# PolarisRisingWar/rgb-experiment

Hardware: AMD Instinct MI355X
Metric: aggregated edges/sec (full-graph GCN d=128, reference epoch = train fwd+bwd+Adam + 2 eval fwd) (higher is better)
Workload: dtype f32

## Files before the change

include/rgbx_hip.h:

```cpp
#ifndef RGBX_HIP_H
#define RGBX_HIP_H

#include <stddef.h>
#include <stdint.h>

#ifdef __cplusplus
extern "C" {
#endif

#define RGBX_VERSION 501

#define RGBX_OK 0
#define RGBX_E_ARG (-1)
#define RGBX_E_RANGE (-2)
#define RGBX_E_ALIGN (-3)
#define RGBX_E_WS (-4)
#define RGBX_E_SHAPE (-5)

typedef void* rgbx_stream_t;

enum {
  RGBX_LOOPS_KEEP = 0,
  RGBX_LOOPS_ADD_REMAINING = 1,
  RGBX_LOOPS_REMOVE_ADD = 2
// ... 100 lines not shown

typedef struct rgbx_spmm_epilogue {
  const struct rgbx_ce_epilogue* ce;
  int64_t n_classes;
  double* out_colsums;
  void* stats_ws;
  size_t stats_ws_bytes;
} rgbx_spmm_epilogue_t;

int rgbx_spmm_csr_epilogue_supported(int64_t d);
int rgbx_spmm_csr_epilogue_f32(const int32_t* rowptr, const int32_t* col, const float* w, const float* rs,
                               const float* x, int64_t ldx, const float* y, int64_t ldy, const float* bias,
                               float* out, int64_t ldo, int64_t N, int64_t d, float a, float b,
                               const rgbx_row_split_t* split, const rgbx_spmm_epilogue_t* epi,
                               rgbx_stream_t stream);

int rgbx_spmm_csr_short_rows_supported(int64_t d);
int rgbx_spmm_csr_short_rows_f32(const int32_t* rowptr, const int32_t* col, const float* w, const float* x, int64_t ldx,
                                 const float* bias, float* out, int64_t ldo, int64_t N, int64_t d, rgbx_stream_t stream);

typedef struct rgbx_ce_epilogue {
  const int64_t* y;
  const uint8_t* mask;
  const float* grad_scale;
  double* stats;
  double* scratch;
  int32_t mask_groups;
  const int32_t* rows;
  int64_t n_rows;
  int32_t skip_unselected;
} rgbx_ce_epilogue_t;

int rgbx_spmm_linear_supported(int64_t K, int64_t Nout, int has_root);
int rgbx_spmm_linear_stats_workspace_bytes(int64_t N, int64_t Nout, size_t* bytes);
int rgbx_spmm_linear_f32(const int32_t* rowptr, const int32_t* col, const float* w, const float* rs,
                         const float* x, int64_t ldx, const float* wt, const float* x_root, int64_t ldr,
                         const float* wt_root, const float* bias, float* out, int64_t ldo, float* z_out,
                         int64_t ldz, const float* pre_scale, const float* pre_shift, const float* pre_rowsum,
                         double* out_colsums, void* stats_ws, size_t stats_ws_bytes,
                         const rgbx_ce_epilogue_t* ce, int64_t N, int64_t K, int64_t Nout,
                         const rgbx_row_split_t* split, rgbx_stream_t stream);

typedef struct rgbx_fused_layer {
  const int32_t* rowptr;
  const int32_t* col;
  const float* w;
  const float* rs;
  const float* x;
  int64_t ldx;
  int64_t x_blk_cols, x_blk_stride;
  const float* wt;
  const float* x_root;
  int64_t ldr;
  int64_t xr_blk_cols, xr_blk_stride;
  const float* wt_root;
  const float* bias;
  float* out;
  int64_t ldo;
  float* out_blk;
  int64_t ob_cols, ob_stride;
  float* z_out;
  int64_t ldz;
  const float* pre_scale;
  const float* pre_shift;
  const float* pre_rowsum;
  double* out_colsums;
// ... 293 lines not shown
```

rgb_experiment_amd/_lib.py:

```python
import ctypes
import os

import torch

_HERE = os.path.dirname(os.path.abspath(__file__))
LIB_PATH = os.path.join(_HERE, "csrc", "librgbx_hip.so")

_P = ctypes.c_void_p
_I64 = ctypes.c_int64
_I = ctypes.c_int
_F = ctypes.c_float

class RowSplit(ctypes.Structure):
    _fields_ = [("threshold", ctypes.c_int32), ("n_chunks", ctypes.c_int32), ("n_long", ctypes.c_int32),
                ("chunk_begin", ctypes.c_void_p), ("chunk_end", ctypes.c_void_p), ("chunk_row", ctypes.c_void_p),
                ("long_row", ctypes.c_void_p),
                ("long_chunk_ptr", ctypes.c_void_p), ("partial", ctypes.c_void_p)]


class MultiOut(ctypes.Structure):
    _fields_ = [(f, t) for name in ("sum", "mean", "var", "std", "max", "argmax", "min", "argmin")
                for f, t in ((name, ctypes.c_void_p), ("ld_" + name, ctypes.c_int64))]


# ... 19 lines not shown
                ("xr_blk_cols", _I64), ("xr_blk_stride", _I64), ("wt_root", _P), ("bias", _P), ("out", _P),
                ("ldo", _I64), ("out_blk", _P), ("ob_cols", _I64), ("ob_stride", _I64), ("z_out", _P), ("ldz", _I64),
                ("pre_scale", _P), ("pre_shift", _P), ("pre_rowsum", _P), ("out_colsums", _P), ("stats_ws", _P),
                ("stats_ws_bytes", ctypes.c_size_t), ("ce", _P), ("N", _I64), ("K", _I64), ("Nout", _I64),
                ("split", _P), ("w_pos", _P), ("z_pos_out", _P), ("col_sel", _P)]


SIGNATURES = {
    "rgbx_csr_workspace_bytes": [_I64, _I64, ctypes.POINTER(ctypes.c_size_t)],
    "rgbx_csr_build": [_P, _P, _I64, _I64, _I, _P, _P, _P, _P, ctypes.c_size_t, _P],
    "rgbx_deg_inv_sqrt_f32": [_P, _I64, _P, _P],
    "rgbx_gcn_norm_f32": [_P, _P, _I64, _P, _P, _P],
    "rgbx_inv_degree_f32": [_P, _I64, _P, _P],
    "rgbx_loop_weights_f32": [_P, _P, _P, _I64, _I64, _I, _F, _P, _P, _P],
    "rgbx_edge_slot_weights_f32": [_P, _I64, _P, _I64, _P, _P, _P],
    "rgbx_weighted_deg_inv_sqrt_f32": [_P, _P, _I64, _P, _P],
    "rgbx_gcn_norm_weighted_f32": [_P, _P, _P, _I64, _P, _P, _P],
    "rgbx_edge_dot_supported": [_I64],
    "rgbx_edge_dot_f32": [_P, _P, _P, _I64, _P, _I64, _P, _I64, _I64, _P, _P],
    "rgbx_gcn_norm_bwd_f32": [_P, _P, _P, _P, _P, _P, _P, _P, _P, _P, _I64, _I64, _P, _P, _P],
    "rgbx_spmm_csr_f32": [_P, _P, _P, _P, _P, _I64, _P, _I64, _P, _P, _I64, _I64, _I64, _F, _F, _P, _P],
    "rgbx_spmm_csr_extremum_supported": [_I64],
    "rgbx_spmm_csr_extremum_f32": [_P, _P, _P, _I64, _P, _I64, _P, _I64, _I64, _I, _P, _P],
    "rgbx_extremum_bwd_f32": [_P, _P, _P, _P, _I64, _P, _P, _I64, _I64, _I64, _P, _P],
    "rgbx_spmm_csr_multi_supported": [_I64],
    "rgbx_spmm_csr_multi_partial_words": [_I64, _I64, _I, ctypes.POINTER(ctypes.c_int64)],
    "rgbx_spmm_csr_multi_f32": [_P, _P, _P, _I64, _P, _I64, _I64, _P, _P],
    "rgbx_multi_bwd_f32": [_P, _P, _P, _P, _P, _I64, _I64, _I64, _P, _P],
    "rgbx_spmm_csr_epilogue_supported": [_I64],
    "rgbx_spmm_csr_epilogue_f32": [_P, _P, _P, _P, _P, _I64, _P, _I64, _P, _P, _I64, _I64, _I64, _F, _F, _P, _P, _P],
    "rgbx_spmm_csr_short_rows_supported": [_I64],
    "rgbx_spmm_csr_short_rows_f32": [_P, _P, _P, _P, _I64, _P, _P, _I64, _I64, _I64, _P],
    "rgbx_spmm_linear_supported": [_I64, _I64, _I],
    "rgbx_spmm_linear_stats_workspace_bytes": [_I64, _I64, ctypes.POINTER(ctypes.c_size_t)],
    "rgbx_spmm_linear_f32": [_P, _P, _P, _P, _P, _I64, _P, _P, _I64, _P, _P, _P, _I64, _P, _I64, _P, _P, _P, _P, _P,
                             ctypes.c_size_t, _P, _I64, _I64, _I64, _P, _P],
    "rgbx_fused_layer_f32": [_P, _P],
    "rgbx_blocked_to_rows_f32": [_P, _I64, _I64, _P, _I64, _I64, _I64, _P, _P],
    "rgbx_appnp_f32": [_P, _P, _P, _P, _I64, _P, _P, _I64, _I64, _I64, _I, _F, _P, _P],
    "rgbx_dagnn_gate_fwd_f32": [_P, _I64, _P, _I64, _I64, _P, _P, _P, _I64, _I64, _I64, _I, _P],
    "rgbx_dagnn_gate_bwd_workspace_bytes": [_I64, ctypes.POINTER(ctypes.c_size_t)],
    "rgbx_dagnn_gate_bwd_f32": [_P, _I64, _P, _I64, _I64, _P, _P, _P, _I64, _P, _I64, _P, _I64, _I64, _P, _P, _P,
                                ctypes.c_size_t, _I64, _I64, _I, _P],
    "rgbx_gru_step_supported": [_I64],
    "rgbx_gru_step_f32": [_P, _P, _P, _I64, _P, _P, _P, _P, _I64, _P, _I64, _P, _I64, _I64, _I64, _P, _P],
    "rgbx_gru_gate_fwd_f32": [_P, _I64, _P, _I64, _P, _I64, _I64, _I64, _P],
    "rgbx_gru_gate_bwd_f32": [_P, _I64, _P, _I64, _P, _I64, _P, _I64, _P, _I64, _I64, _I64, _P],
    "rgbx_gat_scores_f32": [_P, _I64, _P, _P, _P, _P, _I64, _I, _I, _P],
    "rgbx_gat_scores_bwd_scratch_floats": [_I64, _I, _I, ctypes.POINTER(ctypes.c_int64)],
    "rgbx_gat_scores_bwd_f32": [_P, _I64, _P, _P, _I64, _P, _P, _P, _I64, _P, _P, _P, _I64, _I64, _I, _I, _P],
    "rgbx_gat_aggregate_fwd_f32": [_P, _P, _P, _I64, _P, _P, _P, _P, _P, _P, _P, _I64, _P, _P, _P, _P, _I64, _I, _I, _F, _P,
                                   _P],
    "rgbx_gat_edge_softmax_f32": [_P, _P, _P, _P, _F, _P, _P, _P, _P, _P, _I64, _P, _P],
    "rgbx_gat_bwd_dst_f32": [_P, _P, _P, _I64, _P, _P, _P, _P, _P, _I64, _P, _I64, _P, _P, _I64, _I, _I,
                             _F, _P],
    "rgbx_gat_bwd_prep_f32": [_P, _P, _P, _P, _I64, _P, _P, _I64, _P, _P, _P, _F, _P, _I64, _I, _I, _P],
    "rgbx_gat_bwd_src_f32": [_P, _P, _P, _I64, _P, _P, _P, _I64, _P, _I64, _P, _P, _P, _P, _I64, _I, _I, _F, _P, _P],
    "rgbx_supergat_supported": [_I, _I],
    "rgbx_supergat_loss_records": [_I64, _P, ctypes.POINTER(ctypes.c_int64)],
    "rgbx_supergat_aggregate_fwd_f32": [_P, _P, _P, _I64, _P, _P, _P, _P, _I64, _P, _P, _I64, _I, _I, _F, _P, _F, _F, _P,
                                        _I64, _P, _P, _P],
    "rgbx_supergat_bwd_dst_f32": [_P, _P, _P, _I64, _P, _P, _P, _P, _P, _I64, _P, _P, _I64, _P, _P, _I64, _P, _I64, _I, _I,
                                  _F, _P, _F, _F, _P, _P, _P],
    "rgbx_supergat_bwd_src_f32": [_P, _P, _P, _P, _I64, _P, _P, _P, _I64, _P, _I64, _P, _I64, _I, _I, _F, _P, _F, _F, _P,
                                  _P, _P],
    "rgbx_supergat_sample_negatives": [_P, _I64, _I64, _P, _I64, _I, _P, _P, _P],
# ... 122 lines not shown
```

rgb_experiment_amd/csrc/gemm.hip:

```cpp
#include "rgbx_common.h"

namespace rgbx {
namespace {

constexpr int BM = 128, BN = 128, KT = 32;
enum { A_PLAIN = 0, A_BN = 1, A_ROWS = 2 };

struct TnExtra {
  const float* X;
  int64_t ldx;
  const float *mean, *rstd, *ca, *cb, *ck;
  const int32_t* rows;
  int64_t n_rows;
};
using f32x16 = __attribute__((ext_vector_type(16))) float;

template <int W>
__device__ __forceinline__ void stage_tile(float* __restrict__ lds, const float* __restrict__ src,
                                           int64_t ld, int64_t k0, int64_t k_end, int c0, int ncols) {
  const int tid = threadIdx.x;
#pragma unroll 4
  for (int p = 0; p < KT * W / 256; ++p) {
    const int idx = p * 256 + tid;
    const int r = idx / W, c = idx % W;
// ... 20 lines not shown
#pragma unroll
  for (int p = 0; p < KT * (W / 4) / 256; ++p) {
    const int idx = p * 256 + threadIdx.x;
    const int r = idx / (W / 4), c = (idx % (W / 4)) * 4;
    *reinterpret_cast<float4*>(lds + r * W + c) = regs[p];
  }
}

template <int W>
__device__ __forceinline__ void put_tile_bn(float* __restrict__ lds, const float4 (&rg)[KT * (W / 4) / 256],
                                            const float4 (&rx)[KT * (W / 4) / 256], const float* __restrict__ lc,
                                            int64_t k0, int64_t k_end, int c0, int ncols) {
#pragma unroll
  for (int p = 0; p < KT * (W / 4) / 256; ++p) {
    const int idx = p * 256 + threadIdx.x;
    const int r = idx / (W / 4), c = (idx % (W / 4)) * 4;
    float4 v = rg[p];
    if (k0 + r < k_end && c0 + c < ncols) {
      const float4 mu = *reinterpret_cast<const float4*>(lc + 0 * W + c);
      const float4 rs = *reinterpret_cast<const float4*>(lc + 1 * W + c);
      const float4 a = *reinterpret_cast<const float4*>(lc + 2 * W + c);
      const float4 b = *reinterpret_cast<const float4*>(lc + 3 * W + c);
      const float4 k = *reinterpret_cast<const float4*>(lc + 4 * W + c);
      v.x = bn_bwd_input_grad(v.x, rx[p].x, mu.x, rs.x, a.x, b.x, k.x);
      v.y = bn_bwd_input_grad(v.y, rx[p].y, mu.y, rs.y, a.y, b.y, k.y);
      v.z = bn_bwd_input_grad(v.z, rx[p].z, mu.z, rs.z, a.z, b.z, k.z);
      v.w = bn_bwd_input_grad(v.w, rx[p].w, mu.w, rs.w, a.w, b.w, k.w);
    }
    *reinterpret_cast<float4*>(lds + r * W + c) = v;
  }
}

template <int W>
__device__ __forceinline__ void fetch_tile_rows(float4 (&regs)[KT * (W / 4) / 256], const float* __restrict__ src,
                                                int64_t ld, const int32_t* __restrict__ rows, int64_t j0, int64_t j_end,
                                                int c0, int ncols) {
#pragma unroll
  for (int p = 0; p < KT * (W / 4) / 256; ++p) {
    const int idx = p * 256 + threadIdx.x;
    const int r = idx / (W / 4), c = (idx % (W / 4)) * 4;
    const int64_t j = j0 + r;
    regs[p] = make_float4(0.f, 0.f, 0.f, 0.f);
    if (j < j_end && c0 + c < ncols) regs[p] = *reinterpret_cast<const float4*>(src + (int64_t)rows[j] * ld + c0 + c);
  }
}

__device__ __forceinline__ int64_t lower_bound_rows(const int32_t* __restrict__ rows, int64_t n, int64_t key) {
  int64_t lo = 0, hi = n;
  while (lo < hi) {
    const int64_t mid = (lo + hi) >> 1;
    if (rows[mid] < key) lo = mid + 1; else hi = mid;
  }
  return lo;
}

template <bool VEC4, int MT, int MODE = A_PLAIN>
__global__ void __launch_bounds__(256)
gemm_tn_partial_kernel(const float* __restrict__ A, int64_t lda, const float* __restrict__ B, int64_t ldb,
                       float* __restrict__ part, float* __restrict__ colpart, int64_t K, int M, int N,
                       int64_t slab, TnExtra ex) {
  static_assert(MODE == A_PLAIN || VEC4, "the A_BN / A_ROWS forms exist on the 16-byte path only");
  constexpr int MI = MT / 64;
  __shared__ float lds[KT * (MT + 128) + (MODE == A_BN ? 5 * MT : 0)];
  float* la = lds;
  float* lb = lds + KT * MT;
  const int split = blockIdx.x;
  const int m0 = blockIdx.y * MT, n0 = blockIdx.z * BN;
  const int64_t k_begin = (int64_t)split * slab;
  const int64_t k_end = k_begin + slab < K ? k_begin + slab : K;
  const int wave = threadIdx.x >> 6, lane = threadIdx.x & 63;
  const int wm = (wave >> 1) * (MT / 2), wn = (wave & 1) * 64;
  const int kr = lane >> 5, cc = lane & 31;

  f32x16 acc[MI][2];
#pragma unroll
  for (int i = 0; i < MI; ++i)
// ... 20 lines not shown
      for (int i = 0; i < MI; ++i) {
        acc[i][0] = __builtin_amdgcn_mfma_f32_32x32x2f32(a[i], b0, acc[i][0], 0, 0, 0);
        acc[i][1] = __builtin_amdgcn_mfma_f32_32x32x2f32(a[i], b1, acc[i][1], 0, 0, 0);
      }
    }
  };
  if constexpr (MODE == A_BN) {
    float* lc = lds + KT * (MT + 128);
    for (int i = threadIdx.x; i < 5 * MT; i += 256) {
      const float* src = i < MT ? ex.mean : i < 2 * MT ? ex.rstd : i < 3 * MT ? ex.ca : i < 4 * MT ? ex.cb : ex.ck;
      const int c = m0 + i % MT;
      lc[i] = c < M ? src[c] : 0.f;
    }
    float4 ra[KT * (MT / 4) / 256], rx[KT * (MT / 4) / 256], rb[KT * 32 / 256];
    fetch_tile<MT>(ra, A, lda, k_begin, k_end, m0, M);
    fetch_tile<MT>(rx, ex.X, ex.ldx, k_begin, k_end, m0, M);
    fetch_tile<128>(rb, B, ldb, k_begin, k_end, n0, N);
    for (int64_t k0 = k_begin; k0 < k_end; k0 += KT) {
      __syncthreads();
      put_tile_bn<MT>(la, ra, rx, lc, k0, k_end, m0, M);
      put_tile<128>(lb, rb);
      __syncthreads();
      if (k0 + KT < k_end) {
        fetch_tile<MT>(ra, A, lda, k0 + KT, k_end, m0, M);
        fetch_tile<MT>(rx, ex.X, ex.ldx, k0 + KT, k_end, m0, M);
        fetch_tile<128>(rb, B, ldb, k0 + KT, k_end, n0, N);
      }
      consume();
    }
  } else if constexpr (MODE == A_ROWS) {
    const int64_t j_begin = lower_bound_rows(ex.rows, ex.n_rows, k_begin);
    const int64_t j_end = lower_bound_rows(ex.rows, ex.n_rows, k_end);
    float4 ra[KT * (MT / 4) / 256], rb[KT * 32 / 256];
    fetch_tile_rows<MT>(ra, A, lda, ex.rows, j_begin, j_end, m0, M);
    fetch_tile_rows<128>(rb, B, ldb, ex.rows, j_begin, j_end, n0, N);
    for (int64_t j0 = j_begin; j0 < j_end; j0 += KT) {
      __syncthreads();
      put_tile<MT>(la, ra);
      put_tile<128>(lb, rb);
      __syncthreads();
      if (j0 + KT < j_end) {
        fetch_tile_rows<MT>(ra, A, lda, ex.rows, j0 + KT, j_end, m0, M);
        fetch_tile_rows<128>(rb, B, ldb, ex.rows, j0 + KT, j_end, n0, N);
      }
      consume();
    }
  } else if constexpr (VEC4) {
    float4 ra[KT * (MT / 4) / 256], rb[KT * 32 / 256];
    fetch_tile<MT>(ra, A, lda, k_begin, k_end, m0, M);
    fetch_tile<128>(rb, B, ldb, k_begin, k_end, n0, N);
    for (int64_t k0 = k_begin; k0 < k_end; k0 += KT) {
      __syncthreads();
      put_tile<MT>(la, ra);
      put_tile<128>(lb, rb);
      __syncthreads();
      if (k0 + KT < k_end) {
        fetch_tile<MT>(ra, A, lda, k0 + KT, k_end, m0, M);
        fetch_tile<128>(rb, B, ldb, k0 + KT, k_end, n0, N);
      }
      consume();
    }
  } else {
    for (int64_t k0 = k_begin; k0 < k_end; k0 += KT) {
      __syncthreads();
      stage_tile<MT>(la, A, lda, k0, k_end, m0, M);
      stage_tile<128>(lb, B, ldb, k0, k_end, n0, N);
      __syncthreads();
      consume();
    }
  }

  if (sums && m0 + (int)threadIdx.x < M) colpart[(int64_t)split * M + m0 + threadIdx.x] = csum;
  float* out = part + (int64_t)split * M * N;
#pragma unroll
  for (int i = 0; i < MI; ++i)
#pragma unroll
// ... 140 lines not shown
```

rgb_experiment_amd/csrc/spmm_linear.hip:

```cpp
#include "rgbx_common.h"
#include "spmm_internal.h"

namespace rgbx {
namespace {

using f32x16 = __attribute__((ext_vector_type(16))) float;

using f4v = __attribute__((ext_vector_type(4))) float;
__device__ __forceinline__ void nt_store4(float* p, const float (&v)[4]) {
  f4v t = {v[0], v[1], v[2], v[3]};
  __builtin_nontemporal_store(t, reinterpret_cast<f4v*>(p));
}
__device__ __forceinline__ void nt_store1(float* p, float v) { __builtin_nontemporal_store(v, p); }

struct FusedArgs {
  const int* rowptr;
  const int* col;
  const float* w;
  const float* rs;
  const float* x;
  const float* wt;
  const float* xr;
  const float* wtr;
  const float* bias;
  float* out;
  float* z_out;
  int64_t ldx, ldo, ldz, ldr;
  const int* long_row;
  const float* zlong;
  int threshold, n_long;
  int N, K, Nout;
  const float* pre_scale;
  const float* pre_shift;
  const float* pre_rowsum;
  float* stats_part;
  const int64_t* ce_y;
  const uint8_t* ce_mask;
  const float* ce_scale;
  double* ce_part;
  int ce_groups;
  int64_t x_bc, x_bs, xr_bc, xr_bs;
  float* out_blk;
  int64_t ob_c, ob_s;
  const float* w2;
  float* zpos_out;
  const float* zlong_pos;
  const int* ce_rows;
  int ce_n_rows;
  int ce_skip;
  const uint8_t* col_sel;
};

__device__ __forceinline__ const float* blocked_at(const float* base, int64_t bc, int64_t bs, int64_t ld, int row,
                                                   int c) {
  return bc ? base + (int64_t)(c / (int)bc) * bs + (int64_t)row * bc + (c % (int)bc) : base + (int64_t)row * ld + c;
}

constexpr int TM = kTileRows;
constexpr int NT_ROOT = 2;

constexpr int KB = 16;

__device__ __forceinline__ void load_b_batch(float (&b)[KB], const float* __restrict__ wt, int Nout, int n0,
                                             int s0, int kr, int cc) {
#pragma unroll
  for (int i = 0; i < KB; ++i) b[i] = wt[(int64_t)(2 * (s0 + i) + kr) * Nout + n0 + cc];
}

__device__ __forceinline__ void mfma_batch(f32x16& acc, const float (&b)[KB], const float* __restrict__ zt, int ldz,
                                           int s0, int kr, int cc) {
#pragma unroll
  for (int i = 0; i < KB; ++i) {
    const float a = zt[cc * ldz + 2 * (s0 + i) + kr];
    acc = __builtin_amdgcn_mfma_f32_32x32x2f32(a, b[i], acc, 0, 0, 0);
  }
}

template <int KC>
__device__ __forceinline__ void tile_times_wt(f32x16& acc, const float* __restrict__ zt, int ldz,
                                              const float* __restrict__ wt, int K, int Nout, int n0, int kr,
                                              int cc, const float (*first)[KB] = nullptr) {
  if constexpr (KC > 0) {
// ... 98 lines not shown
    for (int b = q; b < G; b += 32) s += part2[(int64_t)b * width2 + c];
  sh[q][j] = s;
  __syncthreads();
  if (q == 0 && c < width2) {
    double t = 0.0;
#pragma unroll
    for (int k = 0; k < 32; ++k) t += sh[k][j];
    sums[c] = t;
  }
}


__device__ __forceinline__ int ce_select(const FusedArgs& A, int row, int* t) {
  int bits = A.ce_mask ? (int)A.ce_mask[row] : 1;
  bits = A.ce_groups == 2 ? (bits & 3) : (bits ? 1 : 0);
  *t = -1;
  if (bits) {
    const int64_t ti = A.ce_y[row];
    if (ti >= 0 && ti < A.Nout) *t = (int)ti;
  }
  return *t >= 0 ? bits : 0;
}

template <bool CE>
__device__ __forceinline__ int tile_row(const FusedArgs& A, int row_base, int r) {
  if constexpr (CE) {
    if (A.ce_rows) {
      const int i = row_base + r;
      const int row = i < A.ce_n_rows ? A.ce_rows[i] : A.N;
      return (unsigned)row < (unsigned)A.N ? row : A.N;
    }
  }
  return row_base + r;
}

__device__ __forceinline__ void ce_epilogue(const FusedArgs& A, const f32x16& acc, float* __restrict__ ot, int row_base,
                                            int wave, int lane, int tile = -1) {
  if (tile < 0) tile = blockIdx.x;
  const int kr = lane >> 5, cc = lane & 31;
  const int ldq = A.Nout + 4;
  const int n0 = wave * 32;
  __syncthreads();
  if (n0 < A.Nout) {
    const float bb = A.bias ? A.bias[n0 + cc] : 0.f;
#pragma unroll
    for (int r = 0; r < 16; ++r) ot[((r & 3) + 8 * (r >> 2) + 4 * kr) * ldq + n0 + cc] = acc[r] + bb;
  }
  __syncthreads();
  double nll = 0.0, nll2 = 0.0;
  int cnt = 0, hit = 0, cnt2 = 0, hit2 = 0;
  const int W = 3 * A.ce_groups;
  const float sc = A.ce_scale ? A.ce_scale[0] : 0.f;
  const bool c0 = lane < A.Nout, c1 = lane + 64 < A.Nout;
  for (int rr = 0; rr < TM / 4; ++rr) {
    const int rl = wave * (TM / 4) + rr;
    const int row = tile_row<true>(A, row_base, rl);
    if (row >= A.N) break;
    int t;
    const int bits = ce_select(A, row, &t);
    if (t < 0 && !A.ce_scale) continue;
    const float v0 = c0 ? ot[rl * ldq + lane] : -INFINITY;
    const float v1 = c1 ? ot[rl * ldq + lane + 64] : -INFINITY;
    float best = v0;
    int arg = c0 ? lane : INT32_MAX;
    if (v1 > best) { best = v1; arg = lane + 64; }
#pragma unroll
    for (int off = 32; off > 0; off >>= 1) {
      const float ob = __shfl_xor(best, off);
      const int oa = __shfl_xor(arg, off);
      if (ob > best || (ob == best && oa < arg)) { best = ob; arg = oa; }
    }
    float se = (c0 ? expf(v0 - best) : 0.f) + (c1 ? expf(v1 - best) : 0.f);
#pragma unroll
    for (int off = 32; off > 0; off >>= 1) se += __shfl_xor(se, off);
    const float lse = best + logf(se);
    if (t >= 0) {
      const double term = (double)(lse - ot[rl * ldq + t]);
      const int h = arg == t ? 1 : 0;
      if (bits & 1) {
        nll += term;
        cnt += 1;
        hit += h;
      }
      if (bits & 2) {
        nll2 += term;
        cnt2 += 1;
        hit2 += h;
      }
    }
    if (A.ce_scale) {
      float* orow = A.out + (int64_t)row * A.ldo;
      if (c0) nt_store1(&orow[lane], t >= 0 ? sc * (expf(v0 - lse) - (lane == t ? 1.f : 0.f)) : 0.f);
      if (c1) nt_store1(&orow[lane + 64], t >= 0 ? sc * (expf(v1 - lse) - (lane + 64 == t ? 1.f : 0.f)) : 0.f);
    }
  }
  __shared__ double cew[4][6];
  if (lane == 0) {
    cew[wave][0] = nll;
    cew[wave][1] = (double)cnt;
    cew[wave][2] = (double)hit;
    cew[wave][3] = nll2;
    cew[wave][4] = (double)cnt2;
    cew[wave][5] = (double)hit2;
  }
  __syncthreads();
  if ((int)threadIdx.x < W) {
    const int k = threadIdx.x;
    A.ce_part[(int64_t)tile * W + k] = (cew[0][k] + cew[1][k]) + (cew[2][k] + cew[3][k]);
  }
}


__device__ __forceinline__ double block_tree_sum(double v, double* sh) {
  sh[threadIdx.x] = v;
  __syncthreads();
  for (int off = 128; off > 0; off >>= 1) {
    if ((int)threadIdx.x < off) sh[threadIdx.x] += sh[threadIdx.x + off];
    __syncthreads();
  }
  const double r = sh[0];
  __syncthreads();
  return r;
}

__global__ void __launch_bounds__(256)
ce_tiles_gather_kernel(const double* __restrict__ part, int n_tiles, double* __restrict__ part2, int W) {
  __shared__ double sh[256];
  const int per = (n_tiles + gridDim.x - 1) / gridDim.x;
  const int b0 = blockIdx.x * per, b1 = min(n_tiles, b0 + per);
  for (int k = 0; k < W; ++k) {
    double v = 0.0;
    for (int b = b0 + threadIdx.x; b < b1; b += 256) v += part[(int64_t)b * W + k];
    v = block_tree_sum(v, sh);
    if (threadIdx.x == 0) part2[blockIdx.x * W + k] = v;
  }
}

__global__ void __launch_bounds__(256)
ce_tiles_finish_kernel(const double* __restrict__ part2, int n, double* __restrict__ stats, int W) {
  __shared__ double sh[256];
  for (int k = 0; k < W; ++k) {
    const double v = block_tree_sum((int)threadIdx.x < n ? part2[threadIdx.x * W + k] : 0.0, sh);
    if (threadIdx.x == 0) stats[k] = v;
  }
}

template <int G, bool HAS_W, int KC, int NT, bool CE = false, bool DENSE = false, bool BLK = false, bool POS = false,
          bool SEL = false>
__global__ void __launch_bounds__(256, POS ? 7 : (NT == 2 ? 5 : 8)) spmm_linear_kernel(const FusedArgs A) {
  constexpr int NG = kWave / G;
  constexpr int U = 4;
  extern __shared__ float zt[];
  const int K = KC ? KC : A.K;
  const int ldz = K + 4;
  const int lane = threadIdx.x & 63, wave = threadIdx.x >> 6;
  const int g = lane / G, t = lane % G;
  const int c = t * 4;
  const bool active = c < K;
  const int row_base = blockIdx.x * TM;

  __shared__ int next_row;
  if constexpr (DENSE) {
    const int k4 = K >> 2;
    for (int idx = threadIdx.x; idx < TM * k4; idx += 256) {
      const int r = idx / k4, c4 = (idx - r * k4) * 4;
      const int row = row_base + r;
      float v[4] = {0.f, 0.f, 0.f, 0.f};
      if (row < A.N) {
        load_vec<4>(v, blocked_at(A.x, BLK ? A.x_bc : 0, A.x_bs, A.ldx, row, c4));
        if (A.pre_scale) {
          float ps[4], pt[4];
          load_vec<4>(ps, A.pre_scale + c4);
          load_vec<4>(pt, A.pre_shift + c4);
          const float rsum = A.pre_rowsum[row];
#pragma unroll
          for (int i = 0; i < 4; ++i) v[i] = fmaf(v[i], ps[i], pt[i] * rsum);
        }
        if (A.z_out) store_vec<4>(A.z_out + (int64_t)row * A.ldz + c4, v);
      }
      store_vec<4>(&zt[r * ldz + c4], v);
    }
  }
  if (!DENSE && threadIdx.x == 0) next_row = 0;
  if constexpr (!DENSE) __syncthreads();
  while (!DENSE) {
    int lr = 0;
    if (lane == 0) lr = atomicAdd(&next_row, 1);
    lr = __builtin_amdgcn_readfirstlane(lr);
    if (lr >= TM) break;
    const int row = tile_row<CE>(A, row_base, lr);
    float acc[4] = {0.f, 0.f, 0.f, 0.f};
    float accp[4] = {0.f, 0.f, 0.f, 0.f};
    bool skip = false;
    if constexpr (CE && !POS) {
      if (A.ce_skip && row < A.N) {
        int t;
        skip = ce_select(A, row, &t) == 0;
      }
    }
    if (row < A.N && !skip) {
      const int start = __builtin_amdgcn_readfirstlane(A.rowptr[row]);
      const int end = __builtin_amdgcn_readfirstlane(A.rowptr[row + 1]);
      if (A.threshold > 0 && end - start > A.threshold) {
        int lo = 0, hi = A.n_long - 1;
        while (lo < hi) {
          const int mid = (lo + hi) >> 1;
          if (A.long_row[mid] < row) lo = mid + 1;
          else hi = mid;
        }
        if (g == 0 && active) {
          load_vec<4>(acc, A.zlong + (int64_t)lo * K + c);
          if constexpr (POS) load_vec<4>(accp, A.zlong_pos + (int64_t)lo * K + c);
        }
      } else {
        const float* xc = A.x + c;
        for (int base = start; base < end; base += kWave) {
          const int n = min(kWave, end - base);
          int mycol = 0;
          float myw = 0.f, mywp = 0.f;
          if (lane < n) {
            mycol = A.col[base + lane];
            if constexpr (HAS_W) myw = A.w[base + lane];
            if constexpr (POS) mywp = A.w2[base + lane];
// ... 472 lines not shown
                                    int64_t ldz, const float* pre_scale, const float* pre_shift,
                                    const float* pre_rowsum, double* out_colsums, void* stats_ws,
                                    size_t stats_ws_bytes, const rgbx_ce_epilogue_t* ce, int64_t N, int64_t K,
                                    int64_t Nout, const rgbx_row_split_t* split, rgbx_stream_t stream) {
  if (!rowptr) return fail(RGBX_E_ARG, "spmm_linear: null pointer");
  rgbx_fused_layer_t L{};
  L.rowptr = rowptr; L.col = col; L.w = w; L.rs = rs; L.x = x; L.ldx = ldx; L.wt = wt;
  L.x_root = x_root; L.ldr = ldr; L.wt_root = wt_root; L.bias = bias; L.out = out; L.ldo = ldo;
  L.z_out = z_out; L.ldz = ldz; L.pre_scale = pre_scale; L.pre_shift = pre_shift; L.pre_rowsum = pre_rowsum;
  L.out_colsums = out_colsums; L.stats_ws = stats_ws; L.stats_ws_bytes = stats_ws_bytes; L.ce = ce;
  L.N = N; L.K = K; L.Nout = Nout; L.split = split;
  return rgbx_fused_layer_f32(&L, stream);
}

extern "C" int rgbx_fused_layer_f32(const rgbx_fused_layer_t* Lp, rgbx_stream_t stream) {
  if (!Lp) return fail(RGBX_E_ARG, "fused_layer: null pointer");
  const rgbx_fused_layer_t& L = *Lp;
  const int64_t N = L.N, K = L.K, Nout = L.Nout;
  const rgbx_ce_epilogue_t* ce = L.ce;
  const bool dense = L.rowptr == nullptr;
  if (N < 0 || K <= 0 || Nout <= 0) return fail(RGBX_E_ARG, "spmm_linear: bad size");
  if (N == 0) return RGBX_OK;
  const bool stats_only = ce && !ce->grad_scale;
  if ((!dense && !L.col) || !L.x || !L.wt || (!L.out && !L.out_blk && !stats_only))
    return fail(RGBX_E_ARG, "spmm_linear: null pointer");
  if (ce) {
    if (!ce->y || !ce->stats || !ce->scratch) return fail(RGBX_E_ARG, "spmm_linear: incomplete cross-entropy epilogue");
    if (Nout > 128) return fail(RGBX_E_SHAPE, "spmm_linear: the cross-entropy epilogue needs Nout <= 128 (got %lld)", (long long)Nout);
    if (L.out_colsums) return fail(RGBX_E_ARG, "spmm_linear: out_colsums and the cross-entropy epilogue exclude each other");
    if (L.out_blk) return fail(RGBX_E_ARG, "spmm_linear: a blocked output and the cross-entropy epilogue exclude each other");
    if (ce->grad_scale && !L.out) return fail(RGBX_E_ARG, "spmm_linear: the loss gradient needs `out`");
    if (ce->mask_groups < 0 || ce->mask_groups > 2)
      return fail(RGBX_E_ARG, "spmm_linear: mask_groups must be 0, 1 or 2 (got %d)", (int)ce->mask_groups);
    if (ce->mask_groups == 2 && (ce->grad_scale || !ce->mask))
      return fail(RGBX_E_ARG, "spmm_linear: two statistics sets (mask_groups == 2) need a mask and no loss gradient");
    if (ce->rows || ce->n_rows) {
      if (!ce->rows || ce->n_rows < 0 || ce->n_rows > N)
        return fail(RGBX_E_ARG, "spmm_linear: row list of %lld rows for N = %lld", (long long)ce->n_rows, (long long)N);
      if (ce->grad_scale || dense || L.z_out || L.w_pos)
        return fail(RGBX_E_ARG, "spmm_linear: a row list needs an aggregating statistics-only launch (no loss gradient, "
                                "no z_out, no w_pos)");
    }
  }
  if (L.col_sel && (dense || ce || L.w_pos || L.out_blk || (L.x_root && L.xr_blk_cols > 0)))
    return fail(RGBX_E_ARG, "fused_layer: col_sel needs an aggregating launch without ce, w_pos or blocked layouts");
  if ((L.w_pos != nullptr) != (L.z_pos_out != nullptr))
    return fail(RGBX_E_ARG, "fused_layer: w_pos and z_pos_out go together");
  if (L.w_pos) {
    if (dense || !L.w || L.rs || L.pre_scale || L.out_blk || L.z_out == nullptr)
      return fail(RGBX_E_ARG, "fused_layer: w_pos needs an aggregating launch with w and z_out, without rs / pre_* / out_blk");
    if ((K != 64 && K != 128 && K != 256) || Nout > 128)
      return fail(RGBX_E_SHAPE, "fused_layer: w_pos needs K in {64, 128, 256} and Nout <= 128 (got K=%lld, Nout=%lld)",
                  (long long)K, (long long)Nout);
    if (!aligned16(L.z_pos_out)) return fail(RGBX_E_ALIGN, "fused_layer: z_pos_out must be 16-byte aligned");
  }
  if (N >= INT32_MAX) return fail(RGBX_E_RANGE, "spmm_linear: N exceeds int32");
  if ((L.x_root != nullptr) != (L.wt_root != nullptr))
    return fail(RGBX_E_ARG, "spmm_linear: x_root and wt_root go together");
  if ((L.pre_scale != nullptr) != (L.pre_shift != nullptr) || (L.pre_scale != nullptr) != (L.pre_rowsum != nullptr))
    return fail(RGBX_E_ARG, "spmm_linear: pre_scale, pre_shift and pre_rowsum go together");
  if (L.pre_scale && (!aligned16(L.pre_scale) || !aligned16(L.pre_shift)))
    return fail(RGBX_E_ALIGN, "spmm_linear: pre_scale / pre_shift must be 16-byte aligned");
  if (!rgbx_spmm_linear_supported(K, Nout, L.x_root != nullptr))
    return fail(RGBX_E_SHAPE,
                "spmm_linear: needs K %% 4 == 0, K <= 256, Nout %% 32 == 0, Nout <= 256 with a root term (got K=%lld, "
                "Nout=%lld)", (long long)K, (long long)Nout);
  const bool x_blk = dense && L.x_blk_cols > 0, xr_blk = L.x_root && L.xr_blk_cols > 0;
  if (!dense && L.x_blk_cols) return fail(RGBX_E_ARG, "fused_layer: a blocked x needs DENSE mode (rowptr == NULL)");
  if (!dense && xr_blk && ((ce && L.w) || L.w_pos))
    return fail(RGBX_E_ARG, "fused_layer: blocked root rows (xr_blk_cols) cannot be combined with per-slot weights plus "
                            "the cross-entropy epilogue, or with w_pos, on an aggregating launch");
  if ((x_blk && (L.x_blk_cols % 4 || L.x_blk_stride % 4 || K % L.x_blk_cols)) ||
      (xr_blk && (L.xr_blk_cols % 4 || L.xr_blk_stride % 4 || K % L.xr_blk_cols)) ||
      (L.out_blk && (L.ob_cols <= 0 || Nout % L.ob_cols)))
// ... 15 lines not shown
    stats_part = reinterpret_cast<float*>(stats_part2 + (size_t)kStatsGather * 2 * Nout);
  }
  hipStream_t s = (hipStream_t)stream;
  const int* long_row = nullptr;
  const float* zlong = nullptr;
  const float* zlong_pos = nullptr;
  int threshold = 0, n_long = 0;
  const rgbx_row_split_t* split = dense ? nullptr : L.split;
  if (split && split->threshold > 0 && split->n_chunks > 0) {
    float* zl = split->partial ? split->partial + (size_t)split->n_chunks * K : nullptr;
    if (int rc = spmm_long_rows_compact(L.rowptr, L.col, L.w, L.rs, L.x, L.ldx, (int)K, split, zl, s)) return rc;
    if (L.w_pos) {
      float* zlp = zl ? zl + (size_t)split->n_long * K : nullptr;
      if (int rc = spmm_long_rows_compact(L.rowptr, L.col, L.w_pos, L.rs, L.x, L.ldx, (int)K, split, zlp, s)) return rc;
      zlong_pos = zlp;
    }
    long_row = split->long_row;
    zlong = zl;
    threshold = split->threshold;
    n_long = split->n_long;
  }
  FusedArgs A{L.rowptr, L.col, L.w, L.rs, L.x, L.wt, L.x_root, L.wt_root, L.bias, L.out, L.z_out,
              L.ldx, L.ldo, L.ldz, L.ldr, long_row, zlong, threshold, n_long, (int)N, (int)K, (int)Nout,
              L.pre_scale, L.pre_shift, L.pre_rowsum, stats_part,
              ce ? ce->y : nullptr, ce ? ce->mask : nullptr, ce ? ce->grad_scale : nullptr, ce ? ce->scratch : nullptr,
              ce && ce->mask_groups == 2 ? 2 : 1,
              x_blk ? L.x_blk_cols : 0, L.x_blk_stride, xr_blk ? L.xr_blk_cols : 0, L.xr_blk_stride,
              L.out_blk, L.ob_cols, L.ob_stride, L.w_pos, L.z_pos_out, zlong_pos};
  A.col_sel = L.col_sel;
  if (ce) {
    A.ce_rows = ce->rows;
    A.ce_n_rows = (int)ce->n_rows;
    A.ce_skip = ce->skip_unselected ? 1 : 0;
  }
  const int64_t tiles = A.ce_rows ? cdiv(A.ce_n_rows, TM) : cdiv(N, TM);
  const int lanes = (int)(K / 4);
  int rc;
  if (dense) {
    if (K == 128 && launch_dense_stream<128>(A, s)) { RGBX_CHECK_LAUNCH("dense_stream_kernel"); rc = RGBX_OK; }
    else if (K == 64 && launch_dense_stream<64>(A, s)) { RGBX_CHECK_LAUNCH("dense_stream_kernel"); rc = RGBX_OK; }
    else if (K == 128) rc = launch<32, 128, true>(A, s);
    else if (K == 64) rc = launch<16, 64, true>(A, s);
    else if (K == 256) rc = launch<64, 256, true>(A, s);
    else rc = launch<32, 0, true>(A, s);
  }
  else if (K == 128) rc = launch<32, 128>(A, s);
  else if (K == 64) rc = launch<16, 64>(A, s);
  else if (K == 256) rc = launch<64, 256>(A, s);
  else if (lanes <= 1) rc = launch<1, 0>(A, s);
  else if (lanes <= 2) rc = launch<2, 0>(A, s);
  else if (lanes <= 4) rc = launch<4, 0>(A, s);
  else if (lanes <= 8) rc = launch<8, 0>(A, s);
  else if (lanes <= 16) rc = launch<16, 0>(A, s);
  else if (lanes <= 32) rc = launch<32, 0>(A, s);
  else rc = launch<64, 0>(A, s);
  if (rc) return rc;
  if (ce) {
    if (int rc2 = reduce_ce_tiles(ce->scratch, (int)tiles, ce->stats, ce->mask_groups == 2 ? 6 : 3, s)) return rc2;
  }
  if (!L.out_colsums) return RGBX_OK;
  return reduce_tile_stats(stats_part, (int)cdiv(N, TM), (int)(2 * Nout), stats_part2, L.out_colsums, N, s);
}

extern "C" int rgbx_spmm_linear_stats_workspace_bytes(int64_t N, int64_t Nout, size_t* bytes) {
  if (!bytes || N < 0 || Nout <= 0) return fail(RGBX_E_ARG, "spmm_linear_stats_workspace_bytes: bad argument");
  *bytes = (size_t)kStatsGather * 2 * (size_t)Nout * sizeof(double) + (size_t)cdiv(N, TM) * 2 * (size_t)Nout * sizeof(float);
  return RGBX_OK;
}
```

rgb_experiment_amd/ops.py:

```python
import ctypes

import torch

from . import _lib

_EVENT_SINK = None


def set_event_sink(sink):
    global _EVENT_SINK
    _EVENT_SINK = sink


class Kind(str):
    variant = None


class _Timed:
    def __init__(self, kind, variant=None):
        if variant is not None and _EVENT_SINK is not None:
            kind = Kind(kind)
            kind.variant = variant
        self.kind = kind

# ... 739 lines not shown
        wtr = wt_root.contiguous()
        keep.append(wtr)
        L.wt_root = wtr.data_ptr()
        if x_root.dim() == 3:
            L.x_root, L.xr_blk_cols, L.xr_blk_stride = _blocked(x_root, "x_root")
        else:
            xr = x_root if x_root.stride(-1) == 1 else x_root.contiguous()
            keep.append(xr)
            L.x_root, L.ldr = xr.data_ptr(), xr.stride(0) if xr.size(0) > 1 else xr.size(1)
    if bias is not None:
        b = bias.contiguous()
        keep.append(b)
        L.bias = b.data_ptr()
    if pre is not None:
        ps, pt, pr = (t.contiguous() for t in pre)
        keep += [ps, pt, pr]
        L.pre_scale, L.pre_shift, L.pre_rowsum = ps.data_ptr(), pt.data_ptr(), pr.data_ptr()
    ce_stats = None
    groups = 1
    if ce is not None:
        y, mask, grad_scale = ce
        if isinstance(mask, (tuple, list)):
            if grad_scale is not None:
                raise RuntimeError("fused_layer: two masks are for statistics only (no loss gradient)")
            mask, groups = group_masks(*mask), 2
        _lib.require_device(y, mask, grad_scale)
        if y.dtype != torch.int64:
            raise RuntimeError(f"labels must be int64, got {y.dtype}")
        if mask is not None and mask.dtype not in (torch.bool, torch.uint8):
            raise RuntimeError(f"mask must be bool, got {mask.dtype}")
        y = y.contiguous()
        mask = None if mask is None else mask.contiguous()
        ce_stats = torch.empty(3 * groups, dtype=torch.float64, device=x.device)
        ce_scratch = torch.empty(3 * groups * ((N + 31) // 32 + 64), dtype=torch.float64, device=x.device)
        ce_arg = _lib.CeEpilogue(_lib.ptr(y), _lib.ptr(mask), _lib.ptr(grad_scale), _lib.ptr(ce_stats),
                                 _lib.ptr(ce_scratch), groups)
        if select_rows and not dense and w_pos is None:
            if grad_scale is not None:
                ce_arg.skip_unselected = 1
            elif not want_z and z is None and mask is not None:
                rows = selected_rows(y, mask, n_out)
                if rows is not None:
                    ce_arg.rows, ce_arg.n_rows = rows.data_ptr(), rows.numel()
                    keep.append(rows)
        keep += [y, mask, ce_scratch, ce_arg]
        L.ce = ctypes.addressof(ce_arg)
        want_out = grad_scale is not None
    if out is not None:
        if tuple(out.shape) != (N, n_out) or out.stride(1) != 1 or out.dtype != torch.float32:
            raise RuntimeError(f"fused_layer: out is {tuple(out.shape)}, expected a float32 [{N}, {n_out}] with contiguous rows")
    elif want_out:
        out = torch.empty((N, n_out), dtype=torch.float32, device=x.device)
    if out is not None:
        L.out, L.ldo = out.data_ptr(), out.stride(0) if N > 1 else n_out
    else:
        L.ldo = n_out
    if out_blocked is not None:
        L.out_blk, L.ob_cols, L.ob_stride = _blocked(out_blocked, "out_blocked")
        if out_blocked.size(1) != N or out_blocked.size(0) * out_blocked.size(2) != n_out:
            raise RuntimeError(f"fused_layer: out_blocked is {tuple(out_blocked.shape)} for a [{N}, {n_out}] output")
    if z is not None:
        if tuple(z.shape) != (N, K) or z.stride(1) != 1 or z.dtype != torch.float32:
            raise RuntimeError(f"fused_layer: z is {tuple(z.shape)}, expected a float32 [{N}, {K}] with contiguous rows")
    elif want_z or w_pos is not None:
        z = torch.empty((N, K), dtype=torch.float32, device=x.device)
    L.ldz = K
    if z is not None:
        L.z_out, L.ldz = z.data_ptr(), z.stride(0) if N > 1 else K
    z_pos = None
    if w_pos is not None:
        _lib.require_device(w_pos)
        z_pos = torch.empty_strided((N, K), (L.ldz, 1), dtype=torch.float32, device=x.device)
        keep.append(w_pos)
        L.w_pos, L.z_pos_out = w_pos.data_ptr(), z_pos.data_ptr()
    colsums = None
    if want_colsums:
        nbytes = ctypes.c_size_t(0)
# ... 79 lines not shown


def aggregate_linear(z, weight, bias=None, root_weight=None, x_root=None, want_colsums=False):
    return _tag_colsums(_AggregateLinear.apply(z, weight, bias, root_weight, x_root, want_colsums), want_colsums)


def fold_bn_linear(weight, bias=None, bias2=None, root_weight=None, bn=None):
    _lib.require_device(weight, bias, bias2, root_weight)
    W = weight.detach()
    W = W if W.stride(-1) == 1 else W.contiguous()
    n_out, K = W.shape
    Wr = None
    if root_weight is not None:
        Wr = root_weight.detach()
        Wr = Wr if Wr.stride(-1) == 1 else Wr.contiguous()
    wt = torch.empty((K, n_out), dtype=torch.float32, device=W.device)
    wrt = torch.empty_like(wt) if Wr is not None else None
    has_b = bias is not None or bias2 is not None or bn is not None
    b_out = torch.empty(n_out, dtype=torch.float32, device=W.device) if has_b else None
    c = lambda t: None if t is None else t.detach().contiguous()
    b1, b2 = c(bias), c(bias2)
    g = be = rm = rv = None
    eps = 0.0
    if bn is not None:
        g, be, rm, rv, eps = c(bn.weight), c(bn.bias), c(bn.running_mean), c(bn.running_var), bn.eps
    _lib.check(_lib.load().rgbx_fold_bn_linear_f32(
        _lib.ptr(W), W.stride(0), _lib.ptr(Wr), 0 if Wr is None else Wr.stride(0), _lib.ptr(b1), _lib.ptr(b2),
        _lib.ptr(g), _lib.ptr(be), _lib.ptr(rm), _lib.ptr(rv), float(eps), _lib.ptr(wt), _lib.ptr(wrt), _lib.ptr(b_out),
        n_out, K, _lib.stream_ptr()), "rgbx_fold_bn_linear_f32")
    return wt, b_out, wrt


FUSE_DENSE_BACKWARD = True

BN_HANDOVER = "_rgbx_bn_handover"


class BNHandover:
    __slots__ = ("bn", "mean", "rstd", "n", "reduce")

    def __init__(self, bn):
        self.bn, self.mean, self.rstd, self.n, self.reduce = bn, None, None, None, None

    def fill(self, mean, rstd, n, reduce):
        self.mean, self.rstd, self.n, self.reduce = mean, rstd, n, reduce


def _take_handover(x, bn):
    rec = getattr(x, BN_HANDOVER, None)
    if rec is None or rec.bn is not bn or rec.mean is not None or not x.requires_grad or not FUSE_DENSE_BACKWARD:
        return None
    return rec


class _PropagateLinear(torch.autograd.Function):

    @staticmethod
    def forward(ctx, x, graph, kind, weight, bias, need_z=True, root_weight=None, x_root=None, want_colsums=False,
                bn_weight=None, bn_bias=None, handover=None):
        x = x.contiguous()
        xr = x if x_root is None else x_root.contiguous()
        w = graph.w if kind == "gcn" else None
        rs = graph.inv_deg if kind == "mean" else None
        if kind not in ("gcn", "mean", "sum"):
            raise ValueError(kind)
        res = spmm_linear_raw(graph.fwd, w, rs, x, weight_t(weight), None if bias is None else bias.detach(),
# ... 1851 lines not shown
```

Before: 17.33 billion.

## Use selected-row lists for loss-gradient CE launches and prefetch GEMM row ids

Lets the fused SpMM+linear+cross-entropy training launch process only the labelled (masked) rows via a row list. Rows that are not listed get zero-filled output and z by the owning waves, and per-row loss and hit records are reduced by a new small kernel. Before, tiles over all N rows were computed and unselected ones skipped. Separately, the row-gathered GEMM now prefetches row indices one tile ahead so the index loads do not serialise with the data loads. The cost is an extra kernel, more scratch space, and zero-fill stores spread across the row-list waves.

```diff
diff --git a/include/rgbx_hip.h b/include/rgbx_hip.h
--- a/include/rgbx_hip.h
+++ b/include/rgbx_hip.h
@@ -156,6 +156,7 @@
 } rgbx_ce_epilogue_t;
 
 int rgbx_spmm_linear_supported(int64_t K, int64_t Nout, int has_root);
+int rgbx_ce_rows_grad_scratch_doubles(int64_t N, int64_t* count);
 int rgbx_spmm_linear_stats_workspace_bytes(int64_t N, int64_t Nout, size_t* bytes);
 int rgbx_spmm_linear_f32(const int32_t* rowptr, const int32_t* col, const float* w, const float* rs,
                          const float* x, int64_t ldx, const float* wt, const float* x_root, int64_t ldr,
diff --git a/rgb_experiment_amd/_lib.py b/rgb_experiment_amd/_lib.py
--- a/rgb_experiment_amd/_lib.py
+++ b/rgb_experiment_amd/_lib.py
@@ -75,6 +75,7 @@
     "rgbx_spmm_csr_short_rows_supported": [_I64],
     "rgbx_spmm_csr_short_rows_f32": [_P, _P, _P, _P, _I64, _P, _P, _I64, _I64, _I64, _P],
     "rgbx_spmm_linear_supported": [_I64, _I64, _I],
+    "rgbx_ce_rows_grad_scratch_doubles": [_I64, ctypes.POINTER(ctypes.c_int64)],
     "rgbx_spmm_linear_stats_workspace_bytes": [_I64, _I64, ctypes.POINTER(ctypes.c_size_t)],
     "rgbx_spmm_linear_f32": [_P, _P, _P, _P, _P, _I64, _P, _P, _I64, _P, _P, _P, _I64, _P, _I64, _P, _P, _P, _P, _P,
                              ctypes.c_size_t, _P, _I64, _I64, _I64, _P, _P],
diff --git a/rgb_experiment_amd/csrc/gemm.hip b/rgb_experiment_amd/csrc/gemm.hip
--- a/rgb_experiment_amd/csrc/gemm.hip
+++ b/rgb_experiment_amd/csrc/gemm.hip
@@ -76,16 +76,23 @@
 }
 
 template <int W>
+__device__ __forceinline__ void fetch_row_ids(int32_t (&ids)[KT * (W / 4) / 256], const int32_t* __restrict__ rows,
+                                              int64_t j0, int64_t j_end) {
+#pragma unroll
+  for (int p = 0; p < KT * (W / 4) / 256; ++p) {
+    const int64_t j = j0 + (p * 256 + (int)threadIdx.x) / (W / 4);
+    ids[p] = j < j_end ? rows[j] : -1;
+  }
+}
+
+template <int W>
 __device__ __forceinline__ void fetch_tile_rows(float4 (&regs)[KT * (W / 4) / 256], const float* __restrict__ src,
-                                                int64_t ld, const int32_t* __restrict__ rows, int64_t j0, int64_t j_end,
-                                                int c0, int ncols) {
-#pragma unroll
-  for (int p = 0; p < KT * (W / 4) / 256; ++p) {
-    const int idx = p * 256 + threadIdx.x;
-    const int r = idx / (W / 4), c = (idx % (W / 4)) * 4;
-    const int64_t j = j0 + r;
+                                                int64_t ld, const int32_t (&ids)[KT * (W / 4) / 256], int c0, int ncols) {
+#pragma unroll
+  for (int p = 0; p < KT * (W / 4) / 256; ++p) {
+    const int c = ((p * 256 + (int)threadIdx.x) % (W / 4)) * 4;
     regs[p] = make_float4(0.f, 0.f, 0.f, 0.f);
-    if (j < j_end && c0 + c < ncols) regs[p] = *reinterpret_cast<const float4*>(src + (int64_t)rows[j] * ld + c0 + c);
+    if (ids[p] >= 0 && c0 + c < ncols) regs[p] = *reinterpret_cast<const float4*>(src + (int64_t)ids[p] * ld + c0 + c);
   }
 }
 
@@ -172,16 +179,23 @@
     const int64_t j_begin = lower_bound_rows(ex.rows, ex.n_rows, k_begin);
     const int64_t j_end = lower_bound_rows(ex.rows, ex.n_rows, k_end);
     float4 ra[KT * (MT / 4) / 256], rb[KT * 32 / 256];
-    fetch_tile_rows<MT>(ra, A, lda, ex.rows, j_begin, j_end, m0, M);
-    fetch_tile_rows<128>(rb, B, ldb, ex.rows, j_begin, j_end, n0, N);
+    int32_t ia[KT * (MT / 4) / 256], ib[KT * 32 / 256];
+    fetch_row_ids<MT>(ia, ex.rows, j_begin, j_end);
+    fetch_row_ids<128>(ib, ex.rows, j_begin, j_end);
+    fetch_tile_rows<MT>(ra, A, lda, ia, m0, M);
+    fetch_tile_rows<128>(rb, B, ldb, ib, n0, N);
+    fetch_row_ids<MT>(ia, ex.rows, j_begin + KT, j_end);
+    fetch_row_ids<128>(ib, ex.rows, j_begin + KT, j_end);
     for (int64_t j0 = j_begin; j0 < j_end; j0 += KT) {
       __syncthreads();
       put_tile<MT>(la, ra);
       put_tile<128>(lb, rb);
       __syncthreads();
       if (j0 + KT < j_end) {
-        fetch_tile_rows<MT>(ra, A, lda, ex.rows, j0 + KT, j_end, m0, M);
-        fetch_tile_rows<128>(rb, B, ldb, ex.rows, j0 + KT, j_end, n0, N);
+        fetch_tile_rows<MT>(ra, A, lda, ia, m0, M);
+        fetch_tile_rows<128>(rb, B, ldb, ib, n0, N);
+        fetch_row_ids<MT>(ia, ex.rows, j0 + 2 * KT, j_end);
+        fetch_row_ids<128>(ib, ex.rows, j0 + 2 * KT, j_end);
       }
       consume();
     }
diff --git a/rgb_experiment_amd/csrc/spmm_linear.hip b/rgb_experiment_amd/csrc/spmm_linear.hip
--- a/rgb_experiment_amd/csrc/spmm_linear.hip
+++ b/rgb_experiment_amd/csrc/spmm_linear.hip
@@ -48,6 +48,8 @@
   const int* ce_rows;
   int ce_n_rows;
   int ce_skip;
+  float* ce_term;
+  uint8_t* ce_hit;
   const uint8_t* col_sel;
 };
 
@@ -212,6 +214,30 @@
     }
   }
   return row_base + r;
+}
+
+__device__ __forceinline__ void zero_rows(float* __restrict__ base, int64_t ld, int q, int lo, int hi, int lane) {
+  const int per = kWave / q, sub = lane / q;
+  const float zero[4] = {0.f, 0.f, 0.f, 0.f};
+  if (sub < per)
+    for (int r = lo + sub; r < hi; r += per) nt_store4(base + (int64_t)r * ld + (lane - sub * q) * 4, zero);
+}
+
+__device__ __forceinline__ void ce_fill_gaps(const FusedArgs& A, int i, int row, int lane) {
+  if (i >= A.ce_n_rows || row >= A.N) return;
+  int lo = 0;
+  if (i > 0) {
+    const int prev = A.ce_rows[i - 1];
+    lo = (unsigned)prev < (unsigned)A.N ? prev + 1 : A.N;
+  }
+  if (lo < row) {
+    zero_rows(A.out, A.ldo, A.Nout >> 2, lo, row, lane);
+    if (A.z_out) zero_rows(A.z_out, A.ldz, A.K >> 2, lo, row, lane);
+  }
+  if (i == A.ce_n_rows - 1 && row + 1 < A.N) {
+    zero_rows(A.out, A.ldo, A.Nout >> 2, row + 1, A.N, lane);
+    if (A.z_out) zero_rows(A.z_out, A.ldz, A.K >> 2, row + 1, A.N, lane);
+  }
 }
 
 __device__ __forceinline__ void ce_epilogue(const FusedArgs& A, const f32x16& acc, float* __restrict__ ot, int row_base,
@@ -254,7 +280,12 @@
 #pragma unroll
     for (int off = 32; off > 0; off >>= 1) se += __shfl_xor(se, off);
     const float lse = best + logf(se);
-    if (t >= 0) {
+    if (t >= 0 && A.ce_term) {
+      if (lane == 0) {
+        A.ce_term[row] = lse - ot[rl * ldq + t];
+        A.ce_hit[row] = arg == t ? 1 : 0;
+      }
+    } else if (t >= 0) {
       const double term = (double)(lse - ot[rl * ldq + t]);
       const int h = arg == t ? 1 : 0;
       if (bits & 1) {
@@ -274,6 +305,7 @@
       if (c1) nt_store1(&orow[lane + 64], t >= 0 ? sc * (expf(v1 - lse) - (lane + 64 == t ? 1.f : 0.f)) : 0.f);
     }
   }
+  if (A.ce_term) return;
   __shared__ double cew[4][6];
   if (lane == 0) {
     cew[wave][0] = nll;
@@ -322,6 +354,33 @@
   for (int k = 0; k < W; ++k) {
     const double v = block_tree_sum((int)threadIdx.x < n ? part2[threadIdx.x * W + k] : 0.0, sh);
     if (threadIdx.x == 0) stats[k] = v;
+  }
+}
+
+__global__ void __launch_bounds__(256) ce_row_records_kernel(const FusedArgs A, int tiles) {
+  const int tid = blockIdx.x * 256 + threadIdx.x;
+  const int b = tid >> 2, w = tid & 3;
+  double v[3] = {0.0, 0.0, 0.0};
+  if (b < tiles) {
+    double nll = 0.0;
+    int cnt = 0, hit = 0;
+    for (int rr = 0; rr < TM / 4; ++rr) {
+      const int row = b * TM + w * (TM / 4) + rr;
+      if (row >= A.N) break;
+      int t;
+      if (ce_select(A, row, &t)) {
+        nll += (double)A.ce_term[row];
+        cnt += 1;
+        hit += A.ce_hit[row];
+      }
+    }
+    v[0] = nll, v[1] = (double)cnt, v[2] = (double)hit;
+  }
+#pragma unroll
+  for (int k = 0; k < 3; ++k) {
+    const double pair = v[k] + __shfl_xor(v[k], 1);
+    const double rec = pair + __shfl_xor(pair, 2);
+    if (w == 0 && b < tiles) A.ce_part[(int64_t)b * 3 + k] = rec;
   }
 }
 
@@ -369,6 +428,9 @@
     lr = __builtin_amdgcn_readfirstlane(lr);
     if (lr >= TM) break;
     const int row = tile_row<CE>(A, row_base, lr);
+    if constexpr (CE && !POS && !DENSE) {
+      if (A.ce_term) ce_fill_gaps(A, row_base + lr, row, lane);
+    }
     float acc[4] = {0.f, 0.f, 0.f, 0.f};
     float accp[4] = {0.f, 0.f, 0.f, 0.f};
     bool skip = false;
@@ -907,14 +969,21 @@
     if (ce->grad_scale && !L.out) return fail(RGBX_E_ARG, "spmm_linear: the loss gradient needs `out`");
     if (ce->mask_groups < 0 || ce->mask_groups > 2)
       return fail(RGBX_E_ARG, "spmm_linear: mask_groups must be 0, 1 or 2 (got %d)", (int)ce->mask_groups);
+    if (ce->mask_groups == 2 && ce->grad_scale && (ce->rows || ce->n_rows))
+      return fail(RGBX_E_ARG, "spmm_linear: a row list with the loss gradient excludes two statistics sets (mask_groups == 2)");
     if (ce->mask_groups == 2 && (ce->grad_scale || !ce->mask))
       return fail(RGBX_E_ARG, "spmm_linear: two statistics sets (mask_groups == 2) need a mask and no loss gradient");
     if (ce->rows || ce->n_rows) {
       if (!ce->rows || ce->n_rows < 0 || ce->n_rows > N)
         return fail(RGBX_E_ARG, "spmm_linear: row list of %lld rows for N = %lld", (long long)ce->n_rows, (long long)N);
-      if (ce->grad_scale || dense || L.z_out || L.w_pos)
-        return fail(RGBX_E_ARG, "spmm_linear: a row list needs an aggregating statistics-only launch (no loss gradient, "
-                                "no z_out, no w_pos)");
+      if (dense || L.w_pos)
+        return fail(RGBX_E_ARG, "spmm_linear: a row list needs an aggregating launch (rowptr set) without w_pos");
+      if (!ce->grad_scale && L.z_out)
+        return fail(RGBX_E_ARG, "spmm_linear: a row list with z_out needs the loss gradient (grad_scale): the "
+                                "statistics-only form leaves unlisted rows unwritten");
+      if (ce->grad_scale && (!aligned16(L.out) || L.ldo % 4))
+        return fail(RGBX_E_ALIGN, "spmm_linear: a row list with the loss gradient needs `out` 16-byte aligned with "
+                                  "ldo %% 4 == 0");
     }
   }
   if (L.col_sel && (dense || ce || L.w_pos || L.out_blk || (L.x_root && L.xr_blk_cols > 0)))
@@ -996,8 +1065,19 @@
     A.ce_rows = ce->rows;
     A.ce_n_rows = (int)ce->n_rows;
     A.ce_skip = ce->skip_unselected ? 1 : 0;
-  }
-  const int64_t tiles = A.ce_rows ? cdiv(A.ce_n_rows, TM) : cdiv(N, TM);
+    if (ce->rows && ce->grad_scale) {
+      if (ce->n_rows == 0) {
+        A.ce_rows = nullptr;
+        A.ce_skip = 1;
+      } else {
+        double* behind = ce->scratch + (size_t)(cdiv(N, TM) + kCeGather) * 3;
+        A.ce_term = reinterpret_cast<float*>(behind);
+        A.ce_hit = reinterpret_cast<uint8_t*>(behind + cdiv(N, 2));
+        A.ce_skip = 0;
+      }
+    }
+  }
+  const int64_t tiles = A.ce_rows && !A.ce_term ? cdiv(A.ce_n_rows, TM) : cdiv(N, TM);
   const int lanes = (int)(K / 4);
   int rc;
   if (dense) {
@@ -1019,11 +1099,21 @@
   else if (lanes <= 32) rc = launch<32, 0>(A, s);
   else rc = launch<64, 0>(A, s);
   if (rc) return rc;
+  if (A.ce_term) {
+    ce_row_records_kernel<<<(int)cdiv(tiles * 4, 256), 256, 0, s>>>(A, (int)tiles);
+    RGBX_CHECK_LAUNCH("ce_row_records_kernel");
+  }
   if (ce) {
     if (int rc2 = reduce_ce_tiles(ce->scratch, (int)tiles, ce->stats, ce->mask_groups == 2 ? 6 : 3, s)) return rc2;
   }
   if (!L.out_colsums) return RGBX_OK;
   return reduce_tile_stats(stats_part, (int)cdiv(N, TM), (int)(2 * Nout), stats_part2, L.out_colsums, N, s);
+}
+
+extern "C" int rgbx_ce_rows_grad_scratch_doubles(int64_t N, int64_t* count) {
+  if (!count || N < 0) return fail(RGBX_E_ARG, "ce_rows_grad_scratch_doubles: bad argument");
+  *count = (cdiv(N, TM) + kCeGather) * 3 + cdiv(N, 2) + cdiv(N, 8);
+  return RGBX_OK;
 }
 
 extern "C" int rgbx_spmm_linear_stats_workspace_bytes(int64_t N, int64_t Nout, size_t* bytes) {
diff --git a/rgb_experiment_amd/ops.py b/rgb_experiment_amd/ops.py
--- a/rgb_experiment_amd/ops.py
+++ b/rgb_experiment_amd/ops.py
@@ -795,17 +795,28 @@
         y = y.contiguous()
         mask = None if mask is None else mask.contiguous()
         ce_stats = torch.empty(3 * groups, dtype=torch.float64, device=x.device)
-        ce_scratch = torch.empty(3 * groups * ((N + 31) // 32 + 64), dtype=torch.float64, device=x.device)
+        scratch_doubles = 3 * groups * ((N + 31) // 32 + 64)
+        rows = None
+        if select_rows and not dense and w_pos is None and mask is not None:
+            if grad_scale is not None:
+                if CE_GRAD_ROW_LIST and (out is None or (out.data_ptr() % 16 == 0 and (N == 1 or out.stride(0) % 4 == 0))):
+                    rows = selected_rows(y, mask, n_out)
+                    if rows is not None and rows.numel() == 0:
+                        rows = None
+            elif not want_z and z is None:
+                rows = selected_rows(y, mask, n_out)
+        if rows is not None and grad_scale is not None:
+            count = ctypes.c_int64(0)
+            _lib.check(lib.rgbx_ce_rows_grad_scratch_doubles(N, ctypes.byref(count)), "rgbx_ce_rows_grad_scratch_doubles")
+            scratch_doubles = count.value
+        ce_scratch = torch.empty(scratch_doubles, dtype=torch.float64, device=x.device)
         ce_arg = _lib.CeEpilogue(_lib.ptr(y), _lib.ptr(mask), _lib.ptr(grad_scale), _lib.ptr(ce_stats),
                                  _lib.ptr(ce_scratch), groups)
-        if select_rows and not dense and w_pos is None:
-            if grad_scale is not None:
-                ce_arg.skip_unselected = 1
-            elif not want_z and z is None and mask is not None:
-                rows = selected_rows(y, mask, n_out)
-                if rows is not None:
-                    ce_arg.rows, ce_arg.n_rows = rows.data_ptr(), rows.numel()
-                    keep.append(rows)
+        if rows is not None:
+            ce_arg.rows, ce_arg.n_rows = rows.data_ptr(), rows.numel()
+            keep.append(rows)
+        elif select_rows and not dense and w_pos is None and grad_scale is not None:
+            ce_arg.skip_unselected = 1
         keep += [y, mask, ce_scratch, ce_arg]
         L.ce = ctypes.addressof(ce_arg)
         want_out = grad_scale is not None
@@ -951,6 +962,7 @@
 
 
 FUSE_DENSE_BACKWARD = True
+CE_GRAD_ROW_LIST = True
 
 BN_HANDOVER = "_rgbx_bn_handover"
 
```

After: 17.64 billion, median of 6. +1.8%, better.
